# clementabary/music2dance

Hardware: AMD Instinct MI355X
Metric: 120-frame seq/sec, phase3 WGAN-GP step, batch 64 per GPU (higher is better)
Workload: dtype f32

## Files before the change

### include/m2d.h

```cpp
#ifndef M2D_H
#define M2D_H
#include <stddef.h>
#ifdef __cplusplus
extern "C" {
#endif

#define M2D_OK 0
#define M2D_ERR_ARG -1
#define M2D_ERR_HIP -2
#define M2D_ERR_WORKSPACE -3
#define M2D_ERR_RANGE -4

const char* m2d_last_error(void);
int m2d_version(void);
int m2d_prof_begin(void);
int m2d_prof_end(double* out, int n_out );
int m2d_prof_dump(char* buf, int cap);
int m2d_plan_model_set(int model);
int m2d_plan_model_get(void);

int m2d_conv1d_fwd(const float* x, const float* w, const float* w_packed, const float* bias, float* y, int B,
                   int Cin, int L, int Cout, int ks, int stride, int pad, int act, float slope,
                   const float* residual, const float* out_mask, float out_mask_slope, double* stats, void* ws,
                   size_t ws_bytes, void* stream);
int m2d_conv1d_bwd_data(const float* dy, const float* w, const float* w_packed, float* dx, int B, int Cin, int L,
                        int Cout, int ks, int stride, int pad, const float* dy_mask, float dy_mask_slope,
                        const float* out_mask, float out_mask_slope, void* ws, size_t ws_bytes, void* stream);
int m2d_conv1d_bwd_weight(const float* x, const float* dy, float* dw, float* dbias, int B, int Cin, int L,
                          int Cout, int ks, int stride, int pad, const float* dy_mask, float dy_mask_slope,
                          void* ws, size_t ws_bytes, void* stream);
int m2d_conv1d_fwd_sum(const float* x, const float* w, const float* w_packed, const float* bias, float* y,
                       float* sum_out, int B, int Cin, int L, int Cout, int ks, int stride, int pad, int act,
                       float slope, const float* residual, const float* out_mask, float out_mask_slope, void* ws,
                       size_t ws_bytes, void* stream);
int m2d_conv1d_k4_applicable(int Cin, int L, int Cout, int ks, int stride, int pad);
size_t m2d_conv1d_k4_packed_elems(int Cout, int Cin, int ks, int pad);
int m2d_conv1d_pack_weights_k4(const float* w, float* out, int Cout, int Cin, int ks, int pad, void* stream);
int m2d_conv1d_fwd_k4(const float* x, const float* w_k4, const float* bias, float* y, float* sum_out, int B, int Cin,
                      int L, int Cout, int ks, int stride, int pad, int act, float slope, const float* residual,
                      const float* out_mask, float out_mask_slope, double* stats, void* ws, size_t ws_bytes,
                      void* stream);
int m2d_conv1d_bwd_data_res(const float* dy, const float* w, const float* w_packed, float* dx, int B, int Cin, int L,
                            int Cout, int ks, int stride, int pad, const float* dy_mask, float dy_mask_slope,
                            const float* residual, const float* out_mask, float out_mask_slope, void* ws,
                            size_t ws_bytes, void* stream);
int m2d_conv1d_bwd_weight_from(const float* x, const float* dy, float* dw, float* dbias, int B, int Cin, int L,
                               int Cout, int ks, int stride, int pad, const float* dy_mask, float dy_mask_slope,
                               int bias_from_sample, void* ws, size_t ws_bytes, void* stream);
int m2d_bn_update_running(const double* sums, double count, float* running_mean, float* running_var, float* tmp, int C,
                          float eps, float momentum, void* stream);
int m2d_conv1d_bwd_data_shared_mask(const float* dy, const float* w, const float* w_packed, float* dx, int B, int Cin,
                                    int L, int Cout, int ks, int stride, int pad, const float* out_mask,
                                    float out_mask_slope, int mask_batch, void* ws, size_t ws_bytes, void* stream);
int m2d_gemm_ld(int mode, const float* a, int lda, const float* b, int ldb, const float* bias, float* c, int ldc,
                int M, int N, int K, int act, float slope, const float* a_mask, float a_mask_slope,
                const float* out_mask, float out_mask_slope, void* ws, size_t ws_bytes, void* stream);
int m2d_tanh_fwd(const float* x, float* y, size_t n, void* stream);
int m2d_tanh_bwd(const float* gy, const float* y, float* gx, size_t n, void* stream);
int m2d_tanh_bwd_bwd(const float* g, const float* gy, const float* y, float* g_y, size_t n, void* stream);
int m2d_pose_pack3(const float* real, const float* fake, const float* alpha, float* out, int B, int T, int C,
                   void* stream);
int m2d_wgan_critic_loss(const float* scores, int B, const float* pen0, const float* pen1, float gamma, float* out,
                         void* stream);
int m2d_conv1d_fwd_windows(const float* track, int B, int S, int T, int hop, int window, const float* w,
                           const float* bias, float* y, int Cout, int ks, int stride, int pad, int act, float slope,
                           double* stats, void* ws, size_t ws_bytes, void* stream);
int m2d_conv1d_bwd_weight_windows(const float* track, int B, int S, int T, int hop, int window, const float* dy,
                                  float* dw, float* dbias, int Cout, int ks, int stride, int pad,
                                  const float* dy_mask, float dy_mask_slope, void* ws, size_t ws_bytes, void* stream);
int m2d_conv1d_pack_weights(const float* w, float* w_fwd, float* w_bwd, int Cout, int Cin, int ks, void* stream);
size_t m2d_conv1d_workspace_bytes(int which, int B, int Cin, int L, int Cout, int ks, int stride, int pad);

int m2d_gemm(int mode, const float* a, const float* b, const float* bias, float* c, int M, int N, int K,
             int act, float slope, const float* a_mask, float a_mask_slope, const float* out_mask,
             float out_mask_slope, void* ws, size_t ws_bytes, void* stream);
size_t m2d_gemm_workspace_bytes(int mode, int M, int N, int K);
int m2d_stream_scratch_set(void* stream, void* zeroed, size_t bytes);
int m2d_stream_create(void** stream);

size_t m2d_bn_workspace_bytes(int C);
size_t m2d_bn_scratch_bytes(int C);
int m2d_bn_fwd(const float* x, const float* gamma, const float* beta, float* running_mean,
               float* running_var, float* y, float* save_mean, float* save_invstd, int B, int C, int L,
               float eps, float momentum, int training, int act, float slope, const float* residual, void* ws,
               size_t ws_bytes, void* scratch, void* stream);
int m2d_bn_bwd(const float* dy, const float* x, const float* gamma, const float* beta, const float* save_mean,
               const float* save_invstd, float* dx, float* dgamma, float* dbeta, int B, int C, int L, int act,
               float slope, void* ws, size_t ws_bytes, void* scratch, void* stream);
int m2d_bn_stats(const float* x, double* sums, int B, int C, int L, void* scratch, void* stream);
int m2d_bn_fwd_sums(const float* x, const double* sums, double count, const float* gamma, const float* beta,
                    float* running_mean, float* running_var, float* y, float* save_mean, float* save_invstd, int B,
                    int C, int L, float eps, float momentum, int act, float slope, const float* residual,
                    void* stream);
int m2d_bn_fwd_to(const float* x, const float* gamma, const float* beta, float* running_mean,
                  float* running_var, float* y, float* save_mean, float* save_invstd, int B, int C, int L,
                  float eps, float momentum, int training, int act, float slope, const float* residual, void* ws,
                  size_t ws_bytes, void* scratch, long long y_batch_stride, void* stream);
int m2d_bn_fwd_sums_to(const float* x, const double* sums, double count, const float* gamma, const float* beta,
                       float* running_mean, float* running_var, float* y, float* save_mean, float* save_invstd, int B,
                       int C, int L, float eps, float momentum, int act, float slope, const float* residual,
                       long long y_batch_stride, void* stream);
int m2d_bn_fwd_sums_pool_to(const float* x, const double* sums, double count, const float* gamma, const float* beta,
                            float* running_mean, float* running_var, float* y, float* pooled, float* save_mean,
                            float* save_invstd, int B, int C, int L, float eps, float momentum, int act, float slope,
                            long long y_batch_stride, void* stream);
int m2d_bn_fwd_sums_upsample2_to(const float* x, const double* sums, double count, const float* gamma, const float* beta,
                                 float* running_mean, float* running_var, float* up, float* save_mean, float* save_invstd,
                                 int B, int C, int L, float eps, float momentum, int act, float slope,
                                 long long up_batch_stride, void* stream);
int m2d_bn_bwd_stats(const float* dy, const float* x, const float* gamma, const float* beta, const float* save_mean,
                     const float* save_invstd, double* sums, int B, int C, int L, int act, float slope,
                     void* scratch, void* stream);
int m2d_bn_bwd_sums(const float* dy, const float* x, const float* gamma, const float* beta, const float* save_mean,
                    const float* save_invstd, const double* sums_local, const double* sums_global, double count,
                    float* dx, float* dgamma, float* dbeta, int B, int C, int L, int act, float slope, void* ws,
                    size_t ws_bytes, void* stream);
int m2d_channel_sums(const float* x, const float* mask, float slope, float* out, int B, int C, int L, void* ws,
                     size_t ws_bytes, void* scratch, void* stream);

int m2d_gru_layer_fwd(const float* gi, const float* w_hh_t, const float* b_hh, const int* lengths, float* out,
                      float* r_s, float* z_s, float* n_s, float* hn_s, int B, int T, int H, void* stream);
int m2d_gru_layer_bwd(const float* dout, const float* out, const float* r_s, const float* z_s, const float* n_s,
                      const float* hn_s, const float* w_hh, const int* lengths, float* dgi, float* dgh,
                      float* dh_buf, int B, int T, int H, void* stream);

int m2d_gru_stack_counters(int B, int L);
int m2d_gru_stack_fwd(const float* gi0, const float* const* w_ih_t, const float* const* b_ih,
                      const float* const* w_hh_t, const float* const* b_hh, float* const* out, float* const* saved,
                      const int* lengths, int B, int T, int H, int L, unsigned* counters, void* stream);
int m2d_gru_stack_fwd_state(const float* gi0, const float* const* w_ih_t, const float* const* b_ih,
                            const float* const* w_hh_t, const float* const* b_hh, float* const* out,
                            float* const* saved, const int* lengths, const float* const* h0, float* const* h_n, int B,
                            int T, int H, int L, unsigned* counters, void* stream);
int m2d_gru_persist_error(void);
int m2d_gru_persist_peek(void);
void* m2d_async_fault_word(void);
int m2d_gru_persist_raise(void);
int m2d_fault_fetch(float* dst, void* stream);
int m2d_gru_stack_bwd(const float* dout, const float* const* out, const float* const* saved,
                      const float* const* w_hh, const float* const* w_ih, float* const* dgi, float* const* dgh,
                      float* const* dh_buf, const int* lengths, int B, int T, int H, int L, unsigned* counters,
                      void* stream);

int m2d_gru_small_fwd(const float* gi, const float* w_hh, const float* b_hh, const int* lengths, float* out,
                      float* h_n, float* saved, int B, int T, int H, void* stream);
int m2d_gru_small_bwd(const float* dout, const float* dh_n, const float* out, const float* saved, const float* w_hh,
                      const int* lengths, float* dgi, float* dgh, int B, int T, int H, void* stream);

size_t m2d_cross_entropy_workspace_bytes(int B, int C);
int m2d_cross_entropy_fwd(const float* logits, const long long* labels, float* loss, long long* pred, int B, int C,
                          void* ws, size_t ws_bytes, void* stream);
int m2d_cross_entropy_bwd(const float* logits, const long long* labels, const float* gout, float* dlogits, int B,
                          int C, void* stream);

int m2d_bce_logits_fwd(const float* x, int n0, float t0, int n1, float t1, float* out, float* dx, void* stream);
int m2d_bce_logits_bwd(const float* x, int n0, float t0, int n1, float t1, const float* gout, float* dx,
                       void* stream);

int m2d_gp_interpolate(const float* real, const float* fake, const float* alpha, float* out, int B, int n,
// ... 86 lines not shown
```

### music2dance_amd/_lib.py

```python
import ctypes
import os

_c = ctypes
_F = _c.c_void_p
_I = _c.c_int
_S = _c.c_size_t
_f = _c.c_float
_L = _c.c_long

LIB_PATH = os.environ.get("M2D_LIB") or os.path.join(os.path.dirname(os.path.abspath(__file__)), "lib",
                                                      "libm2d_hip.so")

class AdamItem(_c.Structure):
    _fields_ = [("param", _c.c_void_p), ("grad", _c.c_void_p), ("exp_avg", _c.c_void_p), ("exp_avg_sq", _c.c_void_p),
                ("numel", _c.c_longlong), ("pack_fwd", _c.c_void_p), ("pack_bwd", _c.c_void_p),
                ("cout", _I), ("cin", _I), ("ks", _I), ("reserved", _I)]


SIGNATURES = {
    "m2d_last_error": (_c.c_char_p, []),
    "m2d_version": (_I, []),
    "m2d_prof_begin": (_I, []),
    "m2d_prof_end": (_I, [_c.POINTER(_c.c_double), _I]),
    "m2d_prof_dump": (_I, [_c.c_char_p, _I]),
    "m2d_plan_model_set": (_I, [_I]),
    "m2d_plan_model_get": (_I, []),
    "m2d_conv1d_fwd": (_I, [_F, _F, _F, _F, _F, _I, _I, _I, _I, _I, _I, _I, _I, _f, _F, _F, _f, _F, _F, _S, _F]),
    "m2d_conv1d_bwd_data": (_I, [_F, _F, _F, _F, _I, _I, _I, _I, _I, _I, _I, _F, _f, _F, _f, _F, _S, _F]),
    "m2d_conv1d_bwd_weight": (_I, [_F, _F, _F, _F, _I, _I, _I, _I, _I, _I, _I, _F, _f, _F, _S, _F]),
    "m2d_conv1d_fwd_sum": (_I, [_F, _F, _F, _F, _F, _F, _I, _I, _I, _I, _I, _I, _I, _I, _f, _F, _F, _f, _F, _S, _F]),
    "m2d_conv1d_k4_applicable": (_I, [_I, _I, _I, _I, _I, _I]),
    "m2d_conv1d_k4_packed_elems": (_S, [_I, _I, _I, _I]),
    "m2d_conv1d_pack_weights_k4": (_I, [_F, _F, _I, _I, _I, _I, _F]),
    "m2d_conv1d_fwd_k4": (_I, [_F, _F, _F, _F, _F, _I, _I, _I, _I, _I, _I, _I, _I, _f, _F, _F, _f, _F, _F, _S, _F]),
    "m2d_conv1d_bwd_data_res": (_I, [_F, _F, _F, _F, _I, _I, _I, _I, _I, _I, _I, _F, _f, _F, _F, _f, _F, _S, _F]),
    "m2d_conv1d_bwd_weight_from": (_I, [_F, _F, _F, _F, _I, _I, _I, _I, _I, _I, _I, _F, _f, _I, _F, _S, _F]),
    "m2d_bn_update_running": (_I, [_F, _c.c_double, _F, _F, _F, _I, _f, _f, _F]),
    "m2d_conv1d_bwd_data_shared_mask": (_I, [_F, _F, _F, _F, _I, _I, _I, _I, _I, _I, _I, _F, _f, _I, _F, _S, _F]),
    "m2d_gemm_ld": (_I, [_I, _F, _I, _F, _I, _F, _F, _I, _I, _I, _I, _I, _f, _F, _f, _F, _f, _F, _S, _F]),
    "m2d_tanh_fwd": (_I, [_F, _F, _S, _F]),
    "m2d_tanh_bwd": (_I, [_F, _F, _F, _S, _F]),
    "m2d_tanh_bwd_bwd": (_I, [_F, _F, _F, _F, _S, _F]),
    "m2d_pose_pack3": (_I, [_F, _F, _F, _F, _I, _I, _I, _F]),
    "m2d_wgan_critic_loss": (_I, [_F, _I, _F, _F, _f, _F, _F]),
    "m2d_conv1d_fwd_windows": (_I, [_F, _I, _I, _I, _I, _I, _F, _F, _F, _I, _I, _I, _I, _I, _f, _F, _F, _S, _F]),
    "m2d_conv1d_bwd_weight_windows": (_I, [_F, _I, _I, _I, _I, _I, _F, _F, _F, _I, _I, _I, _I, _F, _f, _F, _S, _F]),
    "m2d_conv1d_pack_weights": (_I, [_F, _F, _F, _I, _I, _I, _F]),
    "m2d_conv1d_workspace_bytes": (_S, [_I, _I, _I, _I, _I, _I, _I, _I]),
    "m2d_gemm": (_I, [_I, _F, _F, _F, _F, _I, _I, _I, _I, _f, _F, _f, _F, _f, _F, _S, _F]),
    "m2d_gemm_workspace_bytes": (_S, [_I, _I, _I, _I]),
    "m2d_stream_scratch_set": (_I, [_F, _F, _S]),
    "m2d_stream_create": (_I, [_c.POINTER(_c.c_void_p)]),
    "m2d_bn_workspace_bytes": (_S, [_I]),
    "m2d_bn_scratch_bytes": (_S, [_I]),
    "m2d_bn_fwd": (_I, [_F, _F, _F, _F, _F, _F, _F, _F, _I, _I, _I, _f, _f, _I, _I, _f, _F, _F, _S, _F, _F]),
    "m2d_bn_bwd": (_I, [_F, _F, _F, _F, _F, _F, _F, _F, _F, _I, _I, _I, _I, _f, _F, _S, _F, _F]),
    "m2d_bn_stats": (_I, [_F, _F, _I, _I, _I, _F, _F]),
    "m2d_bn_fwd_sums": (_I, [_F, _F, _c.c_double, _F, _F, _F, _F, _F, _F, _F, _I, _I, _I, _f, _f, _I, _f, _F, _F]),
    "m2d_bn_fwd_to": (_I, [_F, _F, _F, _F, _F, _F, _F, _F, _I, _I, _I, _f, _f, _I, _I, _f, _F, _F, _S, _F, _c.c_longlong, _F]),
    "m2d_bn_fwd_sums_to": (_I, [_F, _F, _c.c_double, _F, _F, _F, _F, _F, _F, _F, _I, _I, _I, _f, _f, _I, _f, _F,
                                _c.c_longlong, _F]),
    "m2d_bn_fwd_sums_pool_to": (_I, [_F, _F, _c.c_double, _F, _F, _F, _F, _F, _F, _F, _F, _I, _I, _I, _f, _f, _I, _f,
                                    _c.c_longlong, _F]),
    "m2d_bn_fwd_sums_upsample2_to": (_I, [_F, _F, _c.c_double, _F, _F, _F, _F, _F, _F, _F, _I, _I, _I, _f, _f, _I, _f,
                                         _c.c_longlong, _F]),
    "m2d_bn_bwd_stats": (_I, [_F, _F, _F, _F, _F, _F, _F, _I, _I, _I, _I, _f, _F, _F]),
    "m2d_bn_bwd_sums": (_I, [_F, _F, _F, _F, _F, _F, _F, _F, _c.c_double, _F, _F, _F, _I, _I, _I, _I, _f, _F, _S, _F]),
    "m2d_channel_sums": (_I, [_F, _F, _f, _F, _I, _I, _I, _F, _S, _F, _F]),
    "m2d_gru_layer_fwd": (_I, [_F, _F, _F, _F, _F, _F, _F, _F, _F, _I, _I, _I, _F]),
    "m2d_gru_layer_bwd": (_I, [_F, _F, _F, _F, _F, _F, _F, _F, _F, _F, _F, _I, _I, _I, _F]),
    "m2d_gru_stack_counters": (_I, [_I, _I]),
    "m2d_gru_stack_fwd": (_I, [_F, _F, _F, _F, _F, _F, _F, _F, _I, _I, _I, _I, _F, _F]),
    "m2d_gru_stack_fwd_state": (_I, [_F, _F, _F, _F, _F, _F, _F, _F, _F, _F, _I, _I, _I, _I, _F, _F]),
    "m2d_gru_persist_error": (_I, []),
    "m2d_gru_persist_peek": (_I, []),
    "m2d_async_fault_word": (_c.c_void_p, []),
    "m2d_gru_persist_raise": (_I, []),
    "m2d_fault_fetch": (_I, [_F, _F]),
    "m2d_gru_stack_bwd": (_I, [_F, _F, _F, _F, _F, _F, _F, _F, _F, _I, _I, _I, _I, _F, _F]),
    "m2d_gru_small_fwd": (_I, [_F, _F, _F, _F, _F, _F, _F, _I, _I, _I, _F]),
    "m2d_gru_small_bwd": (_I, [_F, _F, _F, _F, _F, _F, _F, _F, _I, _I, _I, _F]),
    "m2d_cross_entropy_workspace_bytes": (_S, [_I, _I]),
    "m2d_cross_entropy_fwd": (_I, [_F, _F, _F, _F, _I, _I, _F, _S, _F]),
    "m2d_cross_entropy_bwd": (_I, [_F, _F, _F, _F, _I, _I, _F]),
    "m2d_bce_logits_fwd": (_I, [_F, _I, _f, _I, _f, _F, _F, _F]),
    "m2d_bce_logits_bwd": (_I, [_F, _I, _f, _I, _f, _F, _F, _F]),
    "m2d_gp_interpolate": (_I, [_F, _F, _F, _F, _I, _I, _F]),
    "m2d_gp_penalty_workspace_bytes": (_S, [_I]),
    "m2d_gp_penalty_fwd": (_I, [_F, _F, _F, _I, _I, _I, _F, _S, _F]),
    "m2d_gp_penalty_bwd": (_I, [_F, _F, _F, _F, _I, _I, _I, _F]),
    "m2d_reduce_workspace_bytes": (_S, []),
    "m2d_l1_mean_fwd": (_I, [_F, _F, _F, _S, _F, _S, _F]),
    "m2d_l1_mean_bwd": (_I, [_F, _F, _F, _F, _S, _F]),
    "m2d_tv_mean_fwd": (_I, [_F, _F, _I, _I, _I, _L, _L, _L, _F, _S, _F]),
    "m2d_tv_mean_bwd": (_I, [_F, _F, _F, _I, _I, _I, _L, _L, _L, _F]),
    "m2d_jerk_mean_fwd": (_I, [_F, _F, _I, _I, _I, _L, _L, _L, _F, _S, _F]),
    "m2d_affine_cols": (_I, [_F, _F, _F, _F, _S, _I, _F]),
    "m2d_adam_multi": (_I, [_F, _I, _f, _f, _f, _f, _f, _f, _F, _F]),
    "m2d_maxpool2_fwd": (_I, [_F, _F, _S, _I, _F]),
    "m2d_maxpool2_bwd": (_I, [_F, _F, _F, _S, _I, _F]),
    "m2d_upsample2_fwd": (_I, [_F, _F, _S, _I, _F]),
    "m2d_upsample2_fwd_to": (_I, [_F, _F, _S, _I, _I, _c.c_longlong, _F]),
    "m2d_maxpool2_fwd_from": (_I, [_F, _F, _S, _I, _I, _c.c_longlong, _F]),
    "m2d_upsample2_bwd": (_I, [_F, _F, _S, _I, _F]),
    "m2d_label_concat": (_I, [_F, _F, _F, _F, _I, _I, _I, _I, _I, _I, _F]),
    "m2d_pose_pack3_label": (_I, [_F, _F, _F, _F, _F, _F, _F, _I, _I, _I, _I, _I, _F]),
    "m2d_label_embed_bwd": (_I, [_F, _F, _F, _I, _I, _I, _I, _I, _I, _I, _I, _F]),
    "m2d_dropout": (_I, [_F, _F, _F, _c.c_longlong, _f, _f, _c.c_ulonglong, _c.c_ulonglong, _I, _F]),
    "m2d_randn_frames": (_I, [_F, _c.c_ulonglong, _c.c_longlong, _I, _I, _I, _F]),
    "m2d_render_sticks": (_I, [_F, _L, _I, _I, _F, _F]),
    "m2d_resample_poly": (_I, [_F, _c.c_longlong, _I, _c.c_longlong, _F, _I, _I, _I, _F, _c.c_longlong, _I, _c.c_longlong,
                                _I, _F]),
    "m2d_stft_image_elems": (_S, [_I]),
    "m2d_stft_pack_basis": (_I, [_F, _I, _F, _F]),
    "m2d_stft_bands": (_I, [_F, _c.c_longlong, _I, _I, _c.c_longlong, _I, _I, _I, _F, _F, _I, _F, _F]),
    "m2d_onset_flux": (_I, [_F, _I, _I, _I, _f, _F, _F]),
    "m2d_motion_speed": (_I, [_F, _I, _I, _I, _F, _F]),
    "m2d_beat_align_max_frames": (_I, []),
    "m2d_beat_align": (_I, [_F, _F, _I, _I, _c.c_double, _c.c_double, _c.c_double, _F, _F, _F, _F, _F, _F]),
    "m2d_kinetic_features": (_I, [_F, _I, _I, _I, _c.c_double, _I, _F, _F]),
    "m2d_sym_eig_max_dim": (_I, []),
    "m2d_sym_eig_max_sweeps": (_I, []),
    "m2d_feature_moments": (_I, [_F, _c.c_longlong, _I, _I, _F, _F, _F]),
    "m2d_sym_eig_workspace_bytes": (_S, [_I, _I, _I]),
    "m2d_sym_eig": (_I, [_F, _I, _I, _F, _F, _F, _F, _S, _F]),
    "m2d_frechet_workspace_bytes": (_S, [_I, _I]),
    "m2d_frechet": (_I, [_F, _F, _F, _F, _I, _I, _F, _F, _S, _F]),
    "m2d_pairwise_mean_dist_workspace_bytes": (_S, [_I, _I]),
    "m2d_pairwise_mean_dist": (_I, [_F, _c.c_longlong, _I, _I, _I, _F, _F, _S, _F]),
}

_lib = None

# ... 28 lines not shown
```

### music2dance_amd/build.py

```python
import os
import shutil
import subprocess
import sys
from concurrent.futures import ThreadPoolExecutor

PKG_DIR = os.path.dirname(os.path.abspath(__file__))
CSRC = os.path.join(PKG_DIR, "csrc")
LIB_DIR = os.path.join(PKG_DIR, "lib")
LIB_PATH = os.path.join(LIB_DIR, "libm2d_hip.so")
SOURCES = ["m2d_runtime.hip", "gemm_engine.hip", "conv1d.hip", "tcn.hip", "probe_gemm.hip", "conv1d_thin.hip", "bn.hip", "gru.hip",
           "pointwise.hip", "cond.hip", "render.hip", "resample.hip", "spectral.hip", "distrib.hip"]
STAMPED = ["gemm_engine.hip", "tcn.hip"]
STAMP_LIB_PATH = os.path.join(LIB_DIR, "libm2d_hip_stamp.so")
FLAGS = ["--offload-arch=gfx950", "-O3", "-std=c++17", "-fPIC", "-ffp-contract=off", "-Wall",
         "-Wno-unused-function"] + os.environ.get("M2D_EXTRA_FLAGS", "").split()


def _hipcc():
    exe = shutil.which("hipcc") or "/opt/rocm/bin/hipcc"
    if not os.path.exists(exe):
        raise RuntimeError("hipcc not found: cannot build libm2d_hip.so")
    return exe


def _stale(target, deps):
    if not os.path.exists(target):
        return True
    t = os.path.getmtime(target)
    return any(os.path.getmtime(d) > t for d in deps)


def build(force=False, verbose=True, stamp=True):
    os.makedirs(LIB_DIR, exist_ok=True)
    obj_dir = os.path.join(LIB_DIR, "obj")
    os.makedirs(obj_dir, exist_ok=True)
    hipcc = _hipcc()
    headers = [os.path.join(CSRC, f) for f in os.listdir(CSRC) if f.endswith(".h")]
    jobs = []
    objs = []
    for src in SOURCES:
        s = os.path.join(CSRC, src)
        o = os.path.join(obj_dir, src.replace(".hip", ".o"))
        objs.append(o)
        if force or _stale(o, [s] + headers):
            jobs.append([hipcc] + FLAGS + ["-c", s, "-o", o])

    def run(cmd):
        if verbose:
            print("[m2d build]", " ".join(cmd), flush=True)
        r = subprocess.run(cmd, capture_output=True, text=True)
        if r.returncode != 0:
            raise RuntimeError("hipcc failed:\n%s\n%s" % (" ".join(cmd), r.stderr))
        return r

    sobjs = []
    sjobs = []
    if stamp:
        for src in SOURCES:
            if src in STAMPED:
                s = os.path.join(CSRC, src)
                o = os.path.join(obj_dir, src.replace(".hip", ".stamp.o"))
                sobjs.append(o)
                if force or _stale(o, [s] + headers):
                    sjobs.append([hipcc] + FLAGS + ["-DM2D_STAMP", "-c", s, "-o", o])
            else:
                sobjs.append(os.path.join(obj_dir, src.replace(".hip", ".o")))
    with ThreadPoolExecutor(max_workers=4) as ex:
        list(ex.map(run, jobs + sjobs))
    if force or jobs or _stale(LIB_PATH, objs):
        run([hipcc, "--offload-arch=gfx950", "-shared", "-fPIC", "-o", LIB_PATH] + objs)
    if stamp and (force or jobs or sjobs or _stale(STAMP_LIB_PATH, sobjs)):
        run([hipcc, "--offload-arch=gfx950", "-shared", "-fPIC", "-o", STAMP_LIB_PATH] + sobjs)
    return LIB_PATH


if __name__ == "__main__":
    build(force="--force" in sys.argv, stamp="--no-stamp" not in sys.argv)
    print(LIB_PATH)
```

### music2dance_amd/csrc/conv1d.hip

```cpp
#include "gemm_engine.h"
#include "tcn.h"

static inline int conv_out_len(int L, int ks, int stride, int pad) {
  const int span = L + 2 * pad - ks;
  return span < 0 ? 0 : span / stride + 1;
}

static inline bool fits_i32(long long v) { return v >= 0 && v < 2147483647LL; }

struct M2dWinView {
  int T, S, hop;
};
bool m2d_thin_applicable(int Cin, int Cout, int ks, int stride);
bool m2d_thin_long_applicable(int Cin, int Cout, int ks, int stride, int pad, int L);
size_t m2d_thin_long_stats_ws(int B, int Lout);
int m2d_thin_long_fwd(const float* x, const float* w, const float* bias, float* y, int B, int L, int ks, int stride, int pad,
                      int Lout, int act, float slope, const M2dWinView* wv, double* stats, void* ws, size_t ws_bytes,
                      hipStream_t stream);
size_t m2d_thin_bwd_weight_ws(int B, int Cout, int ks, int Lout);
size_t m2d_thin_fwd_stats_ws(int B, int Lout);
int m2d_thin_fwd(const float* x, const float* w, const float* bias, float* y, int B, int L, int Cout, int ks,
                 int stride, int pad, int Lout, int act, float slope, const float* out_mask, float out_mask_slope,
                 const M2dWinView* wv, double* stats, void* ws, size_t ws_bytes, hipStream_t stream);
int m2d_thin_bwd_data(const float* dy, const float* w, float* dx, int B, int L, int Cout, int ks, int stride,
                      int pad, int Lout, const float* dy_mask, float dy_mask_slope, hipStream_t stream);
int m2d_thin_bwd_weight(const float* x, const float* dy, float* dw, float* dbias, int B, int L, int Cout, int ks,
                        int stride, int pad, int Lout, const float* dy_mask, float dy_mask_slope, void* ws,
                        size_t ws_bytes, const M2dWinView* wv, hipStream_t stream);

static inline bool conv_uses_packed(int Cin) { return Cin >= M2D_BK; }
static inline float fwd_tile_penalty(int stride) { return stride > 1 ? 1.25f : 1.f; }

static void fill_fwd(M2dGemmParams& p, const float* x, const float* w, const float* wp, float* y, int B, int Cin,
                     int L, int Cout, int ks, int stride, int pad, int Lout, const M2dWinView* wv = nullptr) {
  memset(&p, 0, sizeof(p));
  p.M = Cout;
  p.N = B * Lout;
  p.K = Cin * ks;
  p.phases = 1;
  const bool packed = conv_uses_packed(Cin);
  M2dOperand& b = p.B;
  b.base = x;
  b.nbytes = m2d_extent_bytes((long long)B * Cin * L);
  b.nrows = p.N;
  b.rdiv = Lout;
  b.rdiv_inv = 1.f / (float)Lout;
  b.r_hi_stride = Cin * L;
  b.r_lo_stride = stride;
  b.r_off = -pad;
  b.r_pos_mul = stride;
  b.r_pos_off = -pad;
  b.lim = L;
  if (wv && wv->T > 0) {
    b.nbytes = m2d_extent_bytes((long long)(B / wv->T) * wv->S);
    b.r_hi_stride = wv->hop;
    b.rdiv2 = wv->T;
    b.rdiv2_inv = 1.f / (float)wv->T;
    b.r_hi2_stride = wv->S;
  }
  if (packed) {
    p.nhi = ks;
    p.kdiv = Cin;
    p.lo_outer = 1;
    p.small_tile_penalty = fwd_tile_penalty(stride);
    m2d_operand_plain(p.A, wp, Cout, 1, ks * Cout, (long long)Cout * Cin * ks);
    p.A.k_hi_stride = Cout;
    b.k_hi_stride = 1;
    b.k_lo_stride = L;
    b.k_pos_hi = 1;
    b.k_pos_lo = 0;
    b.k_safe_lo = 0;
    b.k_safe_hi = 0x7fffffff;
  } else {
    p.nhi = Cin;
    p.kdiv = ks;
    m2d_operand_plain(p.A, w, Cout, Cin * ks, 1, (long long)Cout * Cin * ks);
    p.A.k_hi_stride = ks;
    b.k_hi_stride = L;
    b.k_lo_stride = 1;
    b.k_pos_hi = 0;
    b.k_pos_lo = 1;
    b.k_safe_lo = pad;
    b.k_safe_hi = L - (Lout - 1) * stride + pad;
// ... 681 lines not shown
                          int Cout, int ks, int stride, int pad, const float* dy_mask, float dy_mask_slope,
                          void* ws, size_t ws_bytes, void* stream) {
  return conv1d_bwd_weight_impl(x, dy, dw, dbias, B, Cin, L, Cout, ks, stride, pad, dy_mask, dy_mask_slope, ws,
                                ws_bytes, stream, nullptr);
}

int m2d_conv1d_bwd_weight_from(const float* x, const float* dy, float* dw, float* dbias, int B, int Cin, int L,
                               int Cout, int ks, int stride, int pad, const float* dy_mask, float dy_mask_slope,
                               int bias_from_sample, void* ws, size_t ws_bytes, void* stream) {
  return conv1d_bwd_weight_impl(x, dy, dw, dbias, B, Cin, L, Cout, ks, stride, pad, dy_mask, dy_mask_slope, ws,
                                ws_bytes, stream, nullptr, bias_from_sample);
}

int m2d_conv1d_bwd_weight_windows(const float* track, int B, int S, int T, int hop, int window, const float* dy,
                                  float* dw, float* dbias, int Cout, int ks, int stride, int pad,
                                  const float* dy_mask, float dy_mask_slope, void* ws, size_t ws_bytes, void* stream) {
  if (B <= 0 || T <= 0 || hop <= 0 || window <= 0 || (long long)(T - 1) * hop + window > S)
    M2D_FAIL(M2D_ERR_ARG, "m2d_conv1d_bwd_weight_windows: windows do not fit the track");
  if (!fits_i32((long long)B * S) || !fits_i32((long long)B * T * window))
    M2D_FAIL(M2D_ERR_RANGE, "m2d_conv1d_bwd_weight_windows: tensor exceeds 2^31 elements");
  const M2dWinView wv = {T, S, hop};
  return conv1d_bwd_weight_impl(track, dy, dw, dbias, B * T, 1, window, Cout, ks, stride, pad, dy_mask, dy_mask_slope,
                                ws, ws_bytes, stream, &wv);
}

size_t m2d_conv1d_workspace_bytes(int which, int B, int Cin, int L, int Cout, int ks, int stride, int pad) {
  const int Lout = conv_out_len(L, ks, stride, pad);
  if (Lout <= 0) return 0;
  if (m2d_thin_applicable(Cin, Cout, ks, stride))
    return which == 2 ? m2d_thin_bwd_weight_ws(B, Cout, ks, Lout) : (which == 0 ? m2d_thin_fwd_stats_ws(B, Lout) : 0);
  if (which == 0 && m2d_thin_long_applicable(Cin, Cout, ks, stride, pad, L)) {
    const size_t a = m2d_gemm_plan(Cout, B * Lout, m2d_chunks(Cin, ks), 1, true).ws_bytes + m2d_rowstats_bytes(Cout, B * Lout);
    const size_t t = m2d_thin_long_stats_ws(B, Lout);
    return a > t ? a : t;
  }
  if (which == 0) {
    if (Lout == 1 && pad == 0 && L == ks) {
      const size_t a = m2d_gemm_plan(Cout, B, m2d_chunks(1, Cin * ks), 1, true).ws_bytes, st = m2d_rowstats_bytes(Cout, B);
      return a + st;
    }
    const bool packed = conv_uses_packed(Cin);
    const int nch = packed ? m2d_chunks(ks, Cin) : m2d_chunks(Cin, ks);
    const size_t a = m2d_gemm_plan(Cout, B * Lout, nch, 1, true, packed ? fwd_tile_penalty(stride) : 1.f).ws_bytes;
    const size_t st = m2d_rowstats_bytes(Cout, B * Lout);
    return a + st + (packed ? pack_bytes(Cout, Cin, ks) : 0);
  }
  if (which == 1) {
    if (Lout == 1 && pad == 0 && L == ks) return m2d_gemm_plan(B, Cin * ks, m2d_chunks(1, Cout), 1, true).ws_bytes;
    if (stride == 1) return m2d_gemm_plan(Cin, B * L, m2d_chunks(ks, Cout), 1, true).ws_bytes + pack_bytes(Cout, Cin, ks);
    if (bwd_subpixel(Cin, Cout, ks, stride)) return subpixel_bytes(Cout, Cin, ks, stride) + pack_bytes(Cout, Cin, ks);
    return pack_bytes(Cout, Cin, ks);
  }
  const int nch = Lout >= M2D_BK ? m2d_chunks(B, Lout) : m2d_chunks(Lout, B);
  const int kind = Lout >= M2D_BK ? M2D_PLAN_BWD_WEIGHT : M2D_PLAN_GENERAL;
  const size_t a = m2d_gemm_plan(Cout, Cin * ks, nch, 1, true, 1.0, kind).ws_bytes;
  const size_t c = m2d_gemm_plan(Cout, Cin * ks + 1, nch, 1, true, 1.0, kind).ws_bytes;
  const size_t t = (Lout == L && m2d_tcn_wgrad_applicable(B, Cin, L, Cout, ks, stride, pad)) ? m2d_tcn_wgrad_ws_bytes(B, Cin, L, ks) : 0;
  return (a > c ? a : c) > t ? (a > c ? a : c) : t;
}

static int gemm_impl(int mode, const float* a, int lda, const float* b, int ldb, const float* bias, float* c, int ldc,
                     int M, int N, int K, int act, float slope, const float* a_mask, float a_mask_slope,
                     const float* out_mask, float out_mask_slope, void* ws, size_t ws_bytes, void* stream) {
  if (M < 0 || N < 0 || K < 0 || mode < 0 || mode > 2) M2D_FAIL(M2D_ERR_ARG, "m2d_gemm: bad arguments");
  const int a_cols = mode == 2 ? M : K, b_cols = mode == 0 ? K : N;
  if (lda == 0) lda = a_cols;
  if (ldb == 0) ldb = b_cols;
  if (ldc == 0) ldc = N;
  if (lda < a_cols || ldb < b_cols || ldc < N) M2D_FAIL(M2D_ERR_ARG, "m2d_gemm: leading dimension smaller than the row");
  if (!fits_i32((long long)M * K) || !fits_i32((long long)N * K) || !fits_i32((long long)M * N))
    M2D_FAIL(M2D_ERR_RANGE, "m2d_gemm: matrix exceeds 2^31 elements");
  M2dGemmParams p;
  memset(&p, 0, sizeof(p));
  p.M = M;
  p.N = N;
  p.K = K;
  p.nhi = K > 0 ? 1 : 0;
  p.kdiv = K > 0 ? K : 1;
  p.phases = 1;
  bool akf = true, bkf = true;
  const long long a_rows = mode == 2 ? K : M, b_rows = mode == 0 ? N : K;
  const long long ea = K > 0 ? (a_rows - 1) * lda + a_cols : 1, eb = K > 0 ? (b_rows - 1) * ldb + b_cols : 1;
  if (!fits_i32((long long)(M - 1) * ldc + N)) M2D_FAIL(M2D_ERR_RANGE, "m2d_gemm: output exceeds 2^31 elements");
  if (mode == 0) {
    m2d_operand_plain(p.A, a, M, lda, 1, ea);
    m2d_operand_plain(p.B, b, N, ldb, 1, eb);
    akf = true;
    bkf = true;
  } else if (mode == 1) {
    m2d_operand_plain(p.A, a, M, lda, 1, ea);
    m2d_operand_plain(p.B, b, N, 1, ldb, eb);
    akf = true;
    bkf = false;
  } else {
    m2d_operand_plain(p.A, a, M, 1, lda, ea);
    m2d_operand_plain(p.B, b, N, 1, ldb, eb);
    akf = false;
    bkf = false;
  }
  p.A.mask = a_mask;
  p.A.mask_slope = a_mask_slope;
  m2d_outmap_plain(p.O, c, ldc, 1);
  p.O.bias = bias;
  p.O.bias_mode = bias ? 2 : 0;
  p.O.act = act;
  p.O.slope = slope;
  p.O.mask = out_mask;
  p.O.mask_slope = out_mask_slope;
  return m2d_gemm_launch(p, akf, bkf, true, ws, ws_bytes, (hipStream_t)stream, "m2d_gemm");
}

int m2d_gemm(int mode, const float* a, const float* b, const float* bias, float* c, int M, int N, int K,
             int act, float slope, const float* a_mask, float a_mask_slope, const float* out_mask,
             float out_mask_slope, void* ws, size_t ws_bytes, void* stream) {
  return gemm_impl(mode, a, 0, b, 0, bias, c, 0, M, N, K, act, slope, a_mask, a_mask_slope, out_mask, out_mask_slope,
                   ws, ws_bytes, stream);
}

int m2d_gemm_ld(int mode, const float* a, int lda, const float* b, int ldb, const float* bias, float* c, int ldc,
                int M, int N, int K, int act, float slope, const float* a_mask, float a_mask_slope,
                const float* out_mask, float out_mask_slope, void* ws, size_t ws_bytes, void* stream) {
  return gemm_impl(mode, a, lda, b, ldb, bias, c, ldc, M, N, K, act, slope, a_mask, a_mask_slope, out_mask,
                   out_mask_slope, ws, ws_bytes, stream);
}

size_t m2d_gemm_workspace_bytes(int mode, int M, int N, int K) {
  (void)mode;
  return m2d_gemm_plan(M, N, m2d_chunks(K > 0 ? 1 : 0, K > 0 ? K : 1), 1, true).ws_bytes;
}

}
```

Baseline: 5693.

## Route small and long-K GEMMs to dedicated tiny and split-K MFMA kernels

Adds a small-GEMM path inside the generic GEMM entry point. Tiny problems (small M*N and K up to 256) go to a 64-thread 16x16-tile kernel. Long-K problems with small M and N use a split-K kernel built on 32x32x2 f32 MFMA, which writes per-slab partial sums to workspace and reduces them in a finish kernel that applies the epilogue. The goal is to cut launch and tiling overhead and fill the GPU for shapes the general engine handles poorly. In exchange it adds a second launch and workspace traffic for the long-K path, and the workspace-size query now reports the larger requirement.

```diff
diff --git a/include/m2d.h b/include/m2d.h
--- a/include/m2d.h
+++ b/include/m2d.h
@@ -75,6 +75,8 @@
              int act, float slope, const float* a_mask, float a_mask_slope, const float* out_mask,
              float out_mask_slope, void* ws, size_t ws_bytes, void* stream);
 size_t m2d_gemm_workspace_bytes(int mode, int M, int N, int K);
+int m2d_small_gemm_route(int mode, int M, int N, int K, int lda, int ldb, int ldc, const void* a, const void* b,
+                         const void* c, const void* bias, const void* a_mask, const void* out_mask);
 int m2d_stream_scratch_set(void* stream, void* zeroed, size_t bytes);
 int m2d_stream_create(void** stream);
 
diff --git a/music2dance_amd/_lib.py b/music2dance_amd/_lib.py
--- a/music2dance_amd/_lib.py
+++ b/music2dance_amd/_lib.py
@@ -49,6 +49,7 @@
     "m2d_conv1d_workspace_bytes": (_S, [_I, _I, _I, _I, _I, _I, _I, _I]),
     "m2d_gemm": (_I, [_I, _F, _F, _F, _F, _I, _I, _I, _I, _f, _F, _f, _F, _f, _F, _S, _F]),
     "m2d_gemm_workspace_bytes": (_S, [_I, _I, _I, _I]),
+    "m2d_small_gemm_route": (_I, [_I, _I, _I, _I, _I, _I, _I, _F, _F, _F, _F, _F, _F]),
     "m2d_stream_scratch_set": (_I, [_F, _F, _S]),
     "m2d_stream_create": (_I, [_c.POINTER(_c.c_void_p)]),
     "m2d_bn_workspace_bytes": (_S, [_I]),
diff --git a/music2dance_amd/build.py b/music2dance_amd/build.py
--- a/music2dance_amd/build.py
+++ b/music2dance_amd/build.py
@@ -8,7 +8,7 @@
 CSRC = os.path.join(PKG_DIR, "csrc")
 LIB_DIR = os.path.join(PKG_DIR, "lib")
 LIB_PATH = os.path.join(LIB_DIR, "libm2d_hip.so")
-SOURCES = ["m2d_runtime.hip", "gemm_engine.hip", "conv1d.hip", "tcn.hip", "probe_gemm.hip", "conv1d_thin.hip", "bn.hip", "gru.hip",
+SOURCES = ["m2d_runtime.hip", "gemm_engine.hip", "conv1d.hip", "small_gemm.hip", "tcn.hip", "probe_gemm.hip", "conv1d_thin.hip", "bn.hip", "gru.hip",
            "pointwise.hip", "cond.hip", "render.hip", "resample.hip", "spectral.hip", "distrib.hip"]
 STAMPED = ["gemm_engine.hip", "tcn.hip"]
 STAMP_LIB_PATH = os.path.join(LIB_DIR, "libm2d_hip_stamp.so")
diff --git a/music2dance_amd/csrc/conv1d.hip b/music2dance_amd/csrc/conv1d.hip
--- a/music2dance_amd/csrc/conv1d.hip
+++ b/music2dance_amd/csrc/conv1d.hip
@@ -1,4 +1,5 @@
 #include "gemm_engine.h"
+#include "small_gemm.h"
 #include "tcn.h"
 
 static inline int conv_out_len(int L, int ks, int stride, int pad) {
@@ -846,6 +847,13 @@
   const long long a_rows = mode == 2 ? K : M, b_rows = mode == 0 ? N : K;
   const long long ea = K > 0 ? (a_rows - 1) * lda + a_cols : 1, eb = K > 0 ? (b_rows - 1) * ldb + b_cols : 1;
   if (!fits_i32((long long)(M - 1) * ldc + N)) M2D_FAIL(M2D_ERR_RANGE, "m2d_gemm: output exceeds 2^31 elements");
+  if (m2d_small_gemm_enabled()) {
+    if (const int route = m2d_small_gemm_route(mode, M, N, K, lda, ldb, ldc, a, b, c, bias, a_mask, out_mask)) {
+      const M2dSmallGemm g = {mode, M, N, K, a, b, bias, c, lda, ldb, ldc, act, slope, a_mask, out_mask, a_mask_slope,
+                              out_mask_slope};
+      return m2d_small_gemm_launch(route, g, ws, ws_bytes, (hipStream_t)stream);
+    }
+  }
   if (mode == 0) {
     m2d_operand_plain(p.A, a, M, lda, 1, ea);
     m2d_operand_plain(p.B, b, N, ldb, 1, eb);
@@ -889,8 +897,9 @@
 }
 
 size_t m2d_gemm_workspace_bytes(int mode, int M, int N, int K) {
-  (void)mode;
-  return m2d_gemm_plan(M, N, m2d_chunks(K > 0 ? 1 : 0, K > 0 ? K : 1), 1, true).ws_bytes;
-}
-
-}
+  const size_t e = m2d_gemm_plan(M, N, m2d_chunks(K > 0 ? 1 : 0, K > 0 ? K : 1), 1, true).ws_bytes;
+  const size_t s = m2d_small_gemm_ws_bytes(mode, M, N, K);
+  return e > s ? e : s;
+}
+
+}
diff --git a/music2dance_amd/csrc/small_gemm.h b/music2dance_amd/csrc/small_gemm.h
--- /dev/null
+++ b/music2dance_amd/csrc/small_gemm.h
@@ -0,0 +1,25 @@
+#pragma once
+#include "m2d_common.h"
+
+#define M2D_SG_ENGINE 0
+#define M2D_SG_TINY 1
+#define M2D_SG_LONGK 2
+#define M2D_SG_WIDE 3
+
+struct M2dSmallGemm {
+  int mode, M, N, K;
+  const float *a, *b, *bias;
+  float* c;
+  int lda, ldb, ldc;
+  int act;
+  float slope;
+  const float *a_mask, *out_mask;
+  float a_mask_slope, out_mask_slope;
+};
+
+extern "C" int m2d_small_gemm_route(int mode, int M, int N, int K, int lda, int ldb, int ldc, const void* a,
+                                    const void* b, const void* c, const void* bias, const void* a_mask,
+                                    const void* out_mask);
+size_t m2d_small_gemm_ws_bytes(int mode, int M, int N, int K);
+bool m2d_small_gemm_enabled();
+int m2d_small_gemm_launch(int route, const M2dSmallGemm& g, void* ws, size_t ws_bytes, hipStream_t stream);
diff --git a/music2dance_amd/csrc/small_gemm.hip b/music2dance_amd/csrc/small_gemm.hip
--- /dev/null
+++ b/music2dance_amd/csrc/small_gemm.hip
@@ -0,0 +1,369 @@
+#include "small_gemm.h"
+
+typedef float sg_f4 __attribute__((ext_vector_type(4)));
+typedef float sg_f2 __attribute__((ext_vector_type(2)));
+typedef float sg_f16 __attribute__((ext_vector_type(16)));
+
+static inline bool sg_al16(const void* p) { return ((uintptr_t)p & 15u) == 0; }
+
+#define SG_TINY_MAX_MN 32768
+#define SG_TINY_MAX_K 256
+#define SG_LONG_MAX_MN 256
+#define SG_LONG_MIN_K 2048
+
+extern "C" int m2d_small_gemm_route(int mode, int M, int N, int K, int lda, int ldb, int ldc, const void* a,
+                                    const void* b, const void* c, const void* bias, const void* a_mask,
+                                    const void* out_mask) {
+  (void)c; (void)bias; (void)out_mask; (void)ldc;
+  if (mode < 0 || mode > 2 || M <= 0 || N <= 0 || K < 0) return M2D_SG_ENGINE;
+  if ((long long)M * N <= SG_TINY_MAX_MN && K <= SG_TINY_MAX_K) return M2D_SG_TINY;
+  if (mode == 0 && M <= SG_LONG_MAX_MN && N <= SG_LONG_MAX_MN && K >= SG_LONG_MIN_K) {
+    if (a_mask || !sg_al16(a) || !sg_al16(b) || (lda & 3) || (ldb & 3)) return M2D_SG_ENGINE;
+    return M2D_SG_LONGK;
+  }
+  return M2D_SG_ENGINE;
+}
+
+bool m2d_small_gemm_enabled() {
+  static const bool on = [] { const char* e = getenv("M2D_SMALL_GEMM"); return !(e && e[0] == '0'); }();
+  return on;
+}
+
+#define SG_T 16
+#define SG_KB 128
+#define SG_LD 18
+#define SG_NQ 8
+
+template <bool KF>
+__device__ __forceinline__ void sg_quad_coords(int q, int& s, int& f, int& li, int& ls) {
+  if constexpr (KF) {
+    const int a = q & 7, msub = (q >> 3) & 3, rr = q >> 5;
+    s = (rr >> 2) * 4 + msub;
+    f = ((rr & 3) * 8 + a) * 4;
+    li = f * SG_LD + s;
+    ls = SG_LD;
+  } else {
+    s = q >> 2;
+    f = (q & 3) * 4;
+    li = s * SG_LD + f;
+    ls = 1;
+  }
+}
+
+template <bool VEC>
+__device__ __forceinline__ void sg_load_quad(const float* __restrict__ base, size_t off, int nok, float* x) {
+  if constexpr (VEC) {
+    const sg_f4 t = *reinterpret_cast<const sg_f4*>(base + (nok == 4 ? off : 0));
+#pragma unroll
+    for (int e = 0; e < 4; ++e) x[e] = nok == 4 ? t[e] : 0.f;
+  } else {
+#pragma unroll
+    for (int e = 0; e < 4; ++e) {
+      const float t = base[e < nok ? off + e : 0];
+      x[e] = e < nok ? t : 0.f;
+    }
+  }
+}
+
+template <bool KF, bool VEC, bool MASKED>
+__device__ __forceinline__ void sg_load_panel(const float* __restrict__ base, const float* __restrict__ mask, size_t ld,
+                                              int row0, int R, int k0, int K, int lane, float (*x)[4], float (*mv)[4]) {
+#pragma unroll
+  for (int i = 0; i < SG_NQ; ++i) {
+    int s, f, li, ls;
+    sg_quad_coords<KF>(lane + 64 * i, s, f, li, ls);
+    const int r = row0 + (KF ? s : f), k = k0 + (KF ? f : s);
+    const int left = KF ? (r < R ? K - k : 0) : (k < K ? R - r : 0);
+    const int nok = left >= 4 ? 4 : (left > 0 ? left : 0);
+    const size_t off = KF ? (size_t)r * ld + k : (size_t)k * ld + r;
+    sg_load_quad<VEC>(base, off, nok, x[i]);
+    if constexpr (MASKED) sg_load_quad<VEC>(mask, off, nok, mv[i]);
+  }
+}
+
+template <bool KF, bool MASKED>
+__device__ __forceinline__ void sg_store_panel(float* lds, int lane, const float (*x)[4], const float (*mv)[4],
+                                               float mslope) {
+#pragma unroll
+  for (int i = 0; i < SG_NQ; ++i) {
+    int s, f, li, ls;
+    sg_quad_coords<KF>(lane + 64 * i, s, f, li, ls);
+#pragma unroll
+    for (int e = 0; e < 4; ++e) {
+      float v = x[i][e];
+      if constexpr (MASKED) v *= (mv[i][e] > 0.f ? 1.f : mslope);
+      lds[li + e * ls] = v;
+    }
+  }
+}
+
+template <bool AKF, bool BKF, bool VA, bool VB, bool MASKED>
+__global__ __launch_bounds__(64) void m2d_small_gemm_tiny_kernel(const M2dSmallGemm g) {
+  __shared__ __attribute__((aligned(16))) float lds[2 * SG_KB * SG_LD];
+  float* const As = lds;
+  float* const Bs = lds + SG_KB * SG_LD;
+  const int lane = threadIdx.x, ty = lane >> 3, tx = lane & 7;
+  const int m0 = blockIdx.y * SG_T, n0 = blockIdx.x * SG_T;
+  float ra[SG_NQ][4], rb[SG_NQ][4], rm[SG_NQ][4];
+  float acc[2][2] = {{0.f, 0.f}, {0.f, 0.f}};
+  const int nb = (g.K + SG_KB - 1) / SG_KB;
+  if (nb > 0) {
+    sg_load_panel<AKF, VA, MASKED>(g.a, g.a_mask, (size_t)g.lda, m0, g.M, 0, g.K, lane, ra, rm);
+    sg_load_panel<BKF, VB, false>(g.b, nullptr, (size_t)g.ldb, n0, g.N, 0, g.K, lane, rb, nullptr);
+  }
+  for (int bt = 0; bt < nb; ++bt) {
+    sg_store_panel<AKF, MASKED>(As, lane, ra, rm, g.a_mask_slope);
+    sg_store_panel<BKF, false>(Bs, lane, rb, nullptr, 1.f);
+    __syncthreads();
+    sg_load_panel<AKF, VA, MASKED>(g.a, g.a_mask, (size_t)g.lda, m0, g.M, (bt + 1) * SG_KB, g.K, lane, ra, rm);
+    sg_load_panel<BKF, VB, false>(g.b, nullptr, (size_t)g.ldb, n0, g.N, (bt + 1) * SG_KB, g.K, lane, rb, nullptr);
+    const int kc = g.K - bt * SG_KB < SG_KB ? g.K - bt * SG_KB : SG_KB;
+    const float* ap = As + 2 * ty;
+    const float* bp = Bs + 2 * tx;
+#pragma unroll 8
+    for (int k = 0; k < kc; ++k) {
+      const sg_f2 av = *reinterpret_cast<const sg_f2*>(ap + k * SG_LD);
+      const sg_f2 bv = *reinterpret_cast<const sg_f2*>(bp + k * SG_LD);
+      acc[0][0] = fmaf(av[0], bv[0], acc[0][0]);
+      acc[0][1] = fmaf(av[0], bv[1], acc[0][1]);
+      acc[1][0] = fmaf(av[1], bv[0], acc[1][0]);
+      acc[1][1] = fmaf(av[1], bv[1], acc[1][1]);
+    }
+    __syncthreads();
+  }
+#pragma unroll
+  for (int i = 0; i < 2; ++i)
+#pragma unroll
+    for (int j = 0; j < 2; ++j) {
+      const int row = m0 + 2 * ty + i, col = n0 + 2 * tx + j;
+      if (row < g.M && col < g.N) {
+        const size_t o = (size_t)row * g.ldc + col;
+        float v = acc[i][j];
+        if (g.bias) v += g.bias[col];
+        v = m2d_act(v, g.act, g.slope);
+        if (g.out_mask) v *= (g.out_mask[o] > 0.f ? 1.f : g.out_mask_slope);
+        g.c[o] = v;
+      }
+    }
+}
+
+template <bool AKF, bool BKF>
+static void sg_tiny_launch_mode(const M2dSmallGemm& g, bool va, bool vb, dim3 grid, hipStream_t stream) {
+#define SG_TINY_CASE(VA, VB, MK)                                                                                       \
+  if (va == VA && vb == VB && (g.a_mask != nullptr) == MK)                                                               \
+    hipLaunchKernelGGL((m2d_small_gemm_tiny_kernel<AKF, BKF, VA, VB, MK>), grid, dim3(64), 0, stream, g);
+  SG_TINY_CASE(false, false, false)
+  SG_TINY_CASE(false, true, false)
+  SG_TINY_CASE(true, false, false)
+  SG_TINY_CASE(true, true, false)
+  SG_TINY_CASE(false, false, true)
+  SG_TINY_CASE(false, true, true)
+  SG_TINY_CASE(true, false, true)
+  SG_TINY_CASE(true, true, true)
+#undef SG_TINY_CASE
+}
+
+static void sg_tiny_launch(const M2dSmallGemm& g, hipStream_t stream) {
+  const int a_fast = g.mode == 2 ? g.M : g.K, b_fast = g.mode == 0 ? g.K : g.N;
+  const bool va = sg_al16(g.a) && sg_al16(g.a_mask) && (g.lda & 3) == 0 && a_fast > 0 && (a_fast & 3) == 0;
+  const bool vb = sg_al16(g.b) && (g.ldb & 3) == 0 && b_fast > 0 && (b_fast & 3) == 0;
+  const dim3 grid((unsigned)m2d_ceil_div(g.N, SG_T), (unsigned)m2d_ceil_div(g.M, SG_T));
+  if (g.mode == 0) sg_tiny_launch_mode<true, true>(g, va, vb, grid, stream);
+  else if (g.mode == 1) sg_tiny_launch_mode<true, false>(g, va, vb, grid, stream);
+  else sg_tiny_launch_mode<false, false>(g, va, vb, grid, stream);
+}
+
+#define SG_LM 64
+#define SG_LN 128
+#define SG_LK 32
+
+struct SgLongPlan {
+  int mt, nt, slab, nslab;
+};
+
+static SgLongPlan sg_long_plan(int M, int N, int K) {
+  SgLongPlan pl;
+  pl.mt = m2d_ceil_div(M, SG_LM);
+  pl.nt = m2d_ceil_div(N, SG_LN);
+  int want = 256 / (pl.mt * pl.nt);
+  if (want < 1) want = 1;
+  pl.slab = m2d_ceil_div(m2d_ceil_div(K, want), SG_LK) * SG_LK;
+  pl.nslab = m2d_ceil_div(K, pl.slab);
+  return pl;
+}
+
+struct SgLong {
+  M2dSmallGemm g;
+  float* part;
+  int slab, nslab;
+};
+
+#define SG_LP 36
+#define SG_LROWS (SG_LM + SG_LN)
+#define SG_LQ (SG_LROWS * SG_LK / 4 / 256)
+
+template <bool GUARD>
+__device__ __forceinline__ void sg_long_fetch(const float* const* rowp, int k, int kc, int K, sg_f4* x) {
+#pragma unroll
+  for (int j = 0; j < SG_LQ; ++j) {
+    if constexpr (!GUARD) {
+      x[j] = *reinterpret_cast<const sg_f4*>(rowp[j] + k);
+    } else {
+#pragma unroll
+      for (int e = 0; e < 4; ++e) {
+        const bool in = k + kc + e < K;
+        const float t = rowp[j][in ? k + e : 0];
+        x[j][e] = in ? t : 0.f;
+      }
+    }
+  }
+}
+
+__device__ __forceinline__ void sg_long_stage(float* buf, int t, const sg_f4* x) {
+#pragma unroll
+  for (int j = 0; j < SG_LQ; ++j)
+    *reinterpret_cast<sg_f4*>(buf + ((t >> 3) + 32 * j) * SG_LP + (t & 7) * 4) = x[j];
+}
+
+__device__ __forceinline__ void sg_long_multiply(const float* buf, int w, int i, int h, sg_f16& acc0, sg_f16& acc1) {
+  const float* pa0 = buf + i * SG_LP + 16 * h;
+  const float* pa1 = pa0 + 32 * SG_LP;
+  const float* pb = buf + (SG_LM + 32 * w + i) * SG_LP + 16 * h;
+#pragma unroll
+  for (int u = 0; u < 4; ++u) {
+    const sg_f4 a0 = *reinterpret_cast<const sg_f4*>(pa0 + 4 * u);
+    const sg_f4 a1 = *reinterpret_cast<const sg_f4*>(pa1 + 4 * u);
+    const sg_f4 b = *reinterpret_cast<const sg_f4*>(pb + 4 * u);
+#pragma unroll
+    for (int e = 0; e < 4; ++e) {
+      acc0 = __builtin_amdgcn_mfma_f32_32x32x2f32(a0[e], b[e], acc0, 0, 0, 0);
+      acc1 = __builtin_amdgcn_mfma_f32_32x32x2f32(a1[e], b[e], acc1, 0, 0, 0);
+    }
+  }
+}
+
+template <bool GUARD>
+__device__ __forceinline__ void sg_long_slab(float* lds, const float* const* rowp, int k0, int n, int K, int t, int w, int i,
+                                             int h, sg_f16& acc0, sg_f16& acc1) {
+  float* const buf0 = lds;
+  float* const buf1 = lds + SG_LROWS * SG_LP;
+  sg_f4 r0[SG_LQ], r1[SG_LQ];
+  const int last = k0 + (n - 1) * SG_LK, kc = (t & 7) * 4;
+  auto at = [&](int s) { const int k = k0 + s * SG_LK; return k < last ? k : last; };
+  sg_long_fetch<GUARD>(rowp, at(0), kc, K, r0);
+  sg_long_fetch<GUARD>(rowp, at(1), kc, K, r1);
+  sg_long_stage(buf0, t, r0);
+  __syncthreads();
+  for (int s = 0; s < n; s += 2) {
+    sg_long_fetch<GUARD>(rowp, at(s + 2), kc, K, r0);
+    sg_long_multiply(buf0, w, i, h, acc0, acc1);
+    sg_long_stage(buf1, t, r1);
+    __syncthreads();
+    if (s + 1 >= n) break;
+    sg_long_fetch<GUARD>(rowp, at(s + 3), kc, K, r1);
+    sg_long_multiply(buf1, w, i, h, acc0, acc1);
+    sg_long_stage(buf0, t, r0);
+    __syncthreads();
+  }
+}
+
+__global__ __launch_bounds__(256) void m2d_small_gemm_longk_kernel(const SgLong p) {
+  __shared__ __attribute__((aligned(16))) float lds[2 * SG_LROWS * SG_LP];
+  const M2dSmallGemm& g = p.g;
+  const int t = threadIdx.x, lane = t & 63, w = t >> 6, i = lane & 31, h = lane >> 5;
+  const int s = blockIdx.x, m0 = blockIdx.y * SG_LM, n0 = blockIdx.z * SG_LN;
+  const float* rowp[SG_LQ];
+#pragma unroll
+  for (int j = 0; j < SG_LQ; ++j) {
+    const int r = (t >> 3) + 32 * j;
+    if (r < SG_LM) {
+      const int gr = m0 + r < g.M ? m0 + r : g.M - 1;
+      rowp[j] = g.a + (size_t)gr * g.lda + (t & 7) * 4;
+    } else {
+      const int gr = n0 + r - SG_LM < g.N ? n0 + r - SG_LM : g.N - 1;
+      rowp[j] = g.b + (size_t)gr * g.ldb + (t & 7) * 4;
+    }
+  }
+  sg_f16 acc0, acc1;
+#pragma unroll
+  for (int r = 0; r < 16; ++r) acc0[r] = acc1[r] = 0.f;
+  const int k0 = s * p.slab, n = p.slab / SG_LK;
+  if (k0 + p.slab <= g.K) sg_long_slab<false>(lds, rowp, k0, n, g.K, t, w, i, h, acc0, acc1);
+  else sg_long_slab<true>(lds, rowp, k0, n, g.K, t, w, i, h, acc0, acc1);
+  float* const img = p.part + (size_t)s * g.M * g.N;
+  const int col = n0 + 32 * w + i;
+#pragma unroll
+  for (int r = 0; r < 16; ++r) {
+    const int row = m0 + (r & 3) + 8 * (r >> 2) + 4 * h;
+    if (col < g.N) {
+      if (row < g.M) img[(size_t)row * g.N + col] = acc0[r];
+      if (row + 32 < g.M) img[(size_t)(row + 32) * g.N + col] = acc1[r];
+    }
+  }
+}
+
+#define SG_FW 16
+#define SG_FP 16
+__global__ __launch_bounds__(64 * SG_FW) void m2d_small_gemm_longk_finish_kernel(const SgLong p) {
+  __shared__ float red[SG_FW][64];
+  const M2dSmallGemm& g = p.g;
+  const int t = threadIdx.x & 63, q = threadIdx.x >> 6;
+  const size_t mn = (size_t)g.M * g.N, o = (size_t)blockIdx.x * 64 + t;
+  const int per = (p.nslab + SG_FW - 1) / SG_FW, s0 = q * per;
+  const int cnt = s0 >= p.nslab ? 0 : (s0 + per <= p.nslab ? per : p.nslab - s0);
+  const float* src = p.part + (o < mn ? o : 0) + (size_t)(cnt > 0 ? s0 : 0) * mn;
+  float v[SG_FP];
+#pragma unroll
+  for (int i = 0; i < SG_FP; ++i) v[i] = src[(size_t)(i < cnt ? i : 0) * mn];
+  float sum = 0.f;
+#pragma unroll
+  for (int i = 0; i < SG_FP; ++i) sum += i < cnt ? v[i] : 0.f;
+  red[q][t] = sum;
+  __syncthreads();
+  if (q == 0 && o < mn) {
+    float x = red[0][t];
+#pragma unroll
+    for (int i = 1; i < SG_FW; ++i) x += red[i][t];
+    const int row = (int)(o / g.N), col = (int)(o % g.N);
+    const size_t oc = (size_t)row * g.ldc + col;
+    if (g.bias) x += g.bias[col];
+    x = m2d_act(x, g.act, g.slope);
+    if (g.out_mask) x *= (g.out_mask[oc] > 0.f ? 1.f : g.out_mask_slope);
+    g.c[oc] = x;
+  }
+}
+
+size_t m2d_small_gemm_ws_bytes(int mode, int M, int N, int K) {
+  if (mode != 0 || M <= 0 || N <= 0 || M > SG_LONG_MAX_MN || N > SG_LONG_MAX_MN || K < SG_LONG_MIN_K) return 0;
+  if ((long long)M * N <= SG_TINY_MAX_MN && K <= SG_TINY_MAX_K) return 0;
+  return (size_t)sg_long_plan(M, N, K).nslab * M * N * sizeof(float);
+}
+
+static int sg_long_launch(const M2dSmallGemm& g, void* ws, size_t ws_bytes, hipStream_t stream) {
+  const SgLongPlan pl = sg_long_plan(g.M, g.N, g.K);
+  const size_t need = (size_t)pl.nslab * g.M * g.N * sizeof(float);
+  if (!ws || ws_bytes < need) M2D_FAIL(M2D_ERR_WORKSPACE, "m2d_gemm: K slabs need %zu workspace bytes, got %zu", need, ws_bytes);
+  SgLong p;
+  p.g = g;
+  p.part = (float*)ws;
+  p.slab = pl.slab;
+  p.nslab = pl.nslab;
+  hipLaunchKernelGGL(m2d_small_gemm_longk_kernel, dim3((unsigned)pl.nslab, (unsigned)pl.mt, (unsigned)pl.nt), dim3(256), 0,
+                     stream, p);
+  const unsigned blocks = (unsigned)(((size_t)g.M * g.N + 63) / 64);
+  hipLaunchKernelGGL(m2d_small_gemm_longk_finish_kernel, dim3(blocks), dim3(64 * SG_FW), 0, stream, p);
+  return M2D_OK;
+}
+
+int m2d_small_gemm_launch(int route, const M2dSmallGemm& g, void* ws, size_t ws_bytes, hipStream_t stream) {
+  M2dProfScope prof(M2D_FAM_GEMM, stream, 2.0 * g.M * (double)g.N * g.K, 0.0, "m2d_gemm", g.M, g.N, g.K);
+  if (route == M2D_SG_TINY) {
+    sg_tiny_launch(g, stream);
+  } else if (route == M2D_SG_LONGK) {
+    if (const int rc = sg_long_launch(g, ws, ws_bytes, stream)) return rc;
+  } else {
+    M2D_FAIL(M2D_ERR_ARG, "m2d_gemm: no small-GEMM form %d", route);
+  }
+  M2D_CHECK_LAUNCH("m2d_gemm");
+  return M2D_OK;
+}
```

Result: no change. 5710 (median of 6 runs) (+0.3%).
